# irconde/SSL4POLYP

Hardware: AMD Instinct MI355X
Metric: training-step images/sec/node, ViT-B/16 224^2 (cls fine-tune) (higher is better)
Workload: dtype bf16; 1 GPU; ViT-B/16 classification fine-tune, bs=64/GPU, 224^2, AdamW, random init, finetune mode full (finetune.py:49-91); global_batch=64, parallelism=dp1, launch=eager, lr_schedule=constant

## Files before the change

### ssl4polyp_amd/csrc/pm_attention.hip

```cpp
#include "pm_common.h"
#include <type_traits>

namespace {

template <int DH> constexpr int kTileUnroll = DH == 32 ? 2 : 1;

template <int RB> __device__ __forceinline__ int swz(int row) {
  if constexpr (RB == 64) return (row >> 2) & 3;
  else if constexpr (RB == 128) return (((row >> 1) & 1) << 2) | ((row >> 2) & 3);
  else if constexpr (RB == 384) return row & 7;
  else return row & 15;
}

constexpr int row_bytes_of(int esize, int dh) { return dh == 80 ? (esize == 2 ? 256 : 384) : dh * esize; }
template <typename T, int DH> constexpr int row_bytes() { return row_bytes_of((int)sizeof(T), DH); }

template <typename T, int DH>
__device__ __forceinline__ void load_image(char* img, const T* __restrict__ src, long ld, int rows_valid,
                                           int rows_total, int tid, int nthreads) {
  constexpr int RB = row_bytes<T, DH>();
  constexpr int CPV = DH * sizeof(T) / 16;
  constexpr int CPF = ((DH + 31) / 32) * 32 * sizeof(T) / 16;
  constexpr int EPC = 16 / sizeof(T);
  for (int id = tid; id < rows_total * CPF; id += nthreads) {
    const int row = id / CPF, c = id % CPF;
    u32x4 v = {0u, 0u, 0u, 0u};
    if (row < rows_valid && c < CPV) v = *reinterpret_cast<const u32x4*>(src + (long)row * ld + c * EPC);
    *reinterpret_cast<u32x4*>(img + row * RB + 16 * (c ^ swz<RB>(row))) = v;
  }
}

template <typename T, int DH>
__device__ __forceinline__ Frag16 frag_rows(const char* img, int rb, int kk, int lane) {
  constexpr int RB = row_bytes<T, DH>();
  const int row = rb + (lane & 31);
  const int c = 2 * kk + (lane >> 5);
  Frag16 f;
  f.u = *reinterpret_cast<const u32x4*>(img + row * RB + 16 * (c ^ swz<RB>(row)));
  return f;
}

template <typename T>
__device__ __forceinline__ Frag16 frag_global(const T* __restrict__ rowptr, bool valid, int kk, int lane) {
  constexpr int EPC = 16 / sizeof(T);
  Frag16 f;
  f.u = (u32x4){0u, 0u, 0u, 0u};
  if (valid) f.u = *reinterpret_cast<const u32x4*>(rowptr + (2 * kk + (lane >> 5)) * EPC);
  return f;
}

template <typename T, int DH>
__device__ __forceinline__ f32x16 mma_imgT_acc(const char* PM_LDS_IMAGE img, int rb, int d0, const f32x16& x, f32x16 acc, int lane) {
  constexpr int RB = row_bytes<T, DH>();
  if constexpr (sizeof(T) == 2) {
    const int g = lane >> 4, i = lane & 15, q = i >> 2, p = i & 3, hh = g >> 1;
    const int col = d0 + 16 * (g & 1) + 4 * p;
    const int c = col >> 3, sub = 8 * (p & 1);
    using lds_s4 = __attribute__((address_space(3))) short4v;
#pragma unroll
    for (int s = 0; s < 2; ++s) {
      Frag16 a, b;
      const int r0 = rb + 16 * s + 4 * hh + q;
      const int r1 = r0 + 8;
      const short4v lo = __builtin_amdgcn_ds_read_tr16_b64_v4i16((lds_s4*)(img + r0 * RB + 16 * (c ^ swz<RB>(r0)) + sub));
      const short4v hi = __builtin_amdgcn_ds_read_tr16_b64_v4i16((lds_s4*)(img + r1 * RB + 16 * (c ^ swz<RB>(r1)) + sub));
      a.u[0] = ((unsigned)(unsigned short)lo[0]) | (((unsigned)(unsigned short)lo[1]) << 16);
      a.u[1] = ((unsigned)(unsigned short)lo[2]) | (((unsigned)(unsigned short)lo[3]) << 16);
      a.u[2] = ((unsigned)(unsigned short)hi[0]) | (((unsigned)(unsigned short)hi[1]) << 16);
      a.u[3] = ((unsigned)(unsigned short)hi[2]) | (((unsigned)(unsigned short)hi[3]) << 16);
#pragma unroll
      for (int j = 0; j < 8; ++j) frag_set<T>(b, j, x[8 * s + j]);
      acc = mfma16B<T>(a, b, acc);
    }
  } else {
    const int hh = lane >> 5;
    const int col = d0 + (lane & 31);
#pragma unroll
    for (int r = 0; r < 16; ++r) {
      const int row = rb + acc_row(r, hh);
      const float a = *reinterpret_cast<const float*>(img + row * RB + 16 * ((col >> 2) ^ swz<RB>(row)) + 4 * (col & 3));
      acc = __builtin_amdgcn_mfma_f32_32x32x2f32(a, x[r], acc, 0, 0, 0);
    }
  }
  return acc;
}

__device__ __forceinline__ f32x16 zero16() {
  f32x16 z;
#pragma unroll
  for (int r = 0; r < 16; ++r) z[r] = 0.f;
  return z;
}

template <typename T>
__device__ __forceinline__ void store_tile_T(T* __restrict__ rowptr, bool valid, const f32x16& acc, float scale, int lane,
                                             int ncols = 32) {
  if (!valid) return;
  const int hh = lane >> 5;
#pragma unroll
  for (int g = 0; g < 4; ++g) {
    f32x4 v = {acc[4 * g] * scale, acc[4 * g + 1] * scale, acc[4 * g + 2] * scale, acc[4 * g + 3] * scale};
    if (8 * g + 4 * hh < ncols) store4<T>(rowptr + 8 * g + 4 * hh, v);
  }
}
template <int DH> __device__ __forceinline__ constexpr int tile_cols(int dt) { return DH - 32 * dt < 32 ? DH - 32 * dt : 32; }

constexpr float kLog2e = 1.4426950408889634f;

template <int DH> __device__ __forceinline__ int problem_of_block(int bid, int nprob, int H) {
  if constexpr (DH == 32) {
    if ((nprob & 15) == 0 && (H & 1) == 0) {
      const int xcd = bid & 7, j = bid >> 3;
      return (((j >> 1) << 3) + xcd) * 2 + (j & 1);
    }
  }
  return bid;
}

constexpr int chunk_tiles(int row_bytes, int nt) {
  const int per_tile = 2 * 32 * row_bytes + 2 * 32 * (int)sizeof(float);
  if (nt * per_tile <= 150 * 1024) return nt;
  return (80 * 1024) / per_tile;
}

template <typename T, int DH, int NT, int CT>
__global__ __launch_bounds__(NT * 64) void attn_fwd_kernel(const T* __restrict__ qkv, T* __restrict__ out,
                                                                        float* __restrict__ lse, int N, int H,
                                                                        float scale) {
  constexpr int RB = row_bytes<T, DH>();
  constexpr int KS = DH * sizeof(T) / 32;
  constexpr int DT = (DH + 31) / 32;
  extern __shared__ __attribute__((aligned(16))) char smem[];
  char* imgK = smem;
  char* imgV = smem + CT * 32 * RB;
  const int tid = threadIdx.x, lane = tid & 63, wave = tid >> 6, hh = lane >> 5;
  const int prob = problem_of_block<DH>(blockIdx.x, gridDim.x, H);
  const int b = prob / H, h = prob % H;
  const long ld = 3L * H * DH;
  const T* base = qkv + (long)b * N * ld + h * DH;
  const float c = scale * kLog2e;
  const int q = wave * 32 + (lane & 31);
  const bool qv = q < N;
  Frag16 fq[KS];
  f32x16 o[DT];
#pragma unroll
  for (int dt = 0; dt < DT; ++dt) o[dt] = zero16();
  float m = -INFINITY, l = 0.f;
  for (int c0 = 0; c0 < NT; c0 += CT) {
    if (c0) __syncthreads();
    load_image<T, DH>(imgK, base + H * DH + (long)c0 * 32 * ld, ld, N - c0 * 32, CT * 32, tid, NT * 64);
    load_image<T, DH>(imgV, base + 2 * H * DH + (long)c0 * 32 * ld, ld, N - c0 * 32, CT * 32, tid, NT * 64);
    __syncthreads();
    if (c0 == 0) {
#pragma unroll
      for (int kk = 0; kk < KS; ++kk) fq[kk] = frag_global<T>(base + (long)q * ld, qv, kk, lane);
    }
    const int cend = c0 + CT < NT ? c0 + CT : NT;
#pragma unroll 1
    for (int kt = c0; kt < cend; ++kt) {
      const int rb = (kt - c0) * 32;
      f32x16 s = zero16();
#pragma unroll
      for (int kk = 0; kk < KS; ++kk) s = mfma16B<T>(frag_rows<T, DH>(imgK, rb, kk, lane), fq[kk], s);
      float tm = -INFINITY;
      if (kt * 32 + 32 > N) {
#pragma unroll
        for (int r = 0; r < 16; ++r) {
          const int key = kt * 32 + acc_row(r, hh);
          s[r] = key < N ? s[r] : -INFINITY;
        }
      }
#pragma unroll
      for (int r = 0; r < 16; ++r) tm = fmaxf(tm, s[r]);
      tm = fmaxf(tm, __shfl_xor(tm, 32, 64));
      const float mn = fmaxf(m, tm);
      const float alpha = __builtin_amdgcn_exp2f((m - mn) * c);
      const float mnc = mn * c;
      float ts = 0.f;
#pragma unroll
      for (int r = 0; r < 16; ++r) {
        s[r] = __builtin_amdgcn_exp2f(s[r] * c - mnc);
        ts += s[r];
      }
      l = l * alpha + ts;
      const bool moved = __builtin_amdgcn_ballot_w64(mn != m) != 0;
      m = mn;
#pragma unroll
      for (int dt = 0; dt < DT; ++dt) {
        if (moved) {
#pragma unroll
          for (int r = 0; r < 16; ++r) o[dt][r] *= alpha;
        }
        o[dt] = mma_imgT_acc<T, DH>(imgV, rb, dt * 32, s, o[dt], lane);
      }
    }
  }
  l += __shfl_xor(l, 32, 64);
  if (qv && hh == 0) lse[((long)b * H + h) * N + q] = m * scale + __logf(l);
  const float inv = 1.0f / l;
  T* orow = out + ((long)b * N + q) * H * DH + h * DH;
#pragma unroll
  for (int dt = 0; dt < DT; ++dt) store_tile_T<T>(orow + dt * 32, qv, o[dt], inv, lane, tile_cols<DH>(dt));
}

template <typename T, int DH, int NT, int CT>
__global__ __launch_bounds__(NT * 64) void attn_bwd_q_kernel(const T* __restrict__ qkv, const T* __restrict__ out,
                                                                          const T* __restrict__ dout,
                                                                          const float* __restrict__ lse,
                                                                          float* __restrict__ delta, T* __restrict__ dqkv,
                                                                          int N, int H, float scale) {
  constexpr int RB = row_bytes<T, DH>();
  constexpr int KS = DH * sizeof(T) / 32;
  constexpr int DT = (DH + 31) / 32;
  constexpr int EPC = 16 / sizeof(T);
  extern __shared__ __attribute__((aligned(16))) char smem[];
  char* imgK = smem;
  char* imgV = smem + CT * 32 * RB;
  const int tid = threadIdx.x, lane = tid & 63, wave = tid >> 6, hh = lane >> 5;
  const int prob = problem_of_block<DH>(blockIdx.x, gridDim.x, H);
  const int b = prob / H, h = prob % H;
  const long ld = 3L * H * DH, ldo = (long)H * DH;
  const T* base = qkv + (long)b * N * ld + h * DH;
  const float c = scale * kLog2e;
  const int q = wave * 32 + (lane & 31);
  const bool qv = q < N;
  const long sidx = ((long)b * H + h) * N + q;
  Frag16 fq[KS], fdo[KS];
  float l2 = 0.f, dls = 0.f;
  f32x16 dq[DT];
#pragma unroll
  for (int dt = 0; dt < DT; ++dt) dq[dt] = zero16();
  for (int c0 = 0; c0 < NT; c0 += CT) {
    if (c0) __syncthreads();
    load_image<T, DH>(imgK, base + H * DH + (long)c0 * 32 * ld, ld, N - c0 * 32, CT * 32, tid, NT * 64);
    load_image<T, DH>(imgV, base + 2 * H * DH + (long)c0 * 32 * ld, ld, N - c0 * 32, CT * 32, tid, NT * 64);
    __syncthreads();
    if (c0 == 0) {
      const T* orow = out + ((long)b * N + q) * ldo + h * DH;
      const T* dorow = dout + ((long)b * N + q) * ldo + h * DH;
      float dl = 0.f;
#pragma unroll
      for (int kk = 0; kk < KS; ++kk) {
        fq[kk] = frag_global<T>(base + (long)q * ld, qv, kk, lane);
        fdo[kk] = frag_global<T>(dorow, qv, kk, lane);
        const Frag16 fo = frag_global<T>(orow, qv, kk, lane);
#pragma unroll
        for (int e = 0; e < EPC; ++e) dl += frag_get<T>(fdo[kk], e) * frag_get<T>(fo, e);
      }
      dl += __shfl_xor(dl, 32, 64);
      if (qv && hh == 0) delta[sidx] = dl;
      l2 = qv ? lse[sidx] * kLog2e : 0.f;
      dls = dl * scale;
    }
    const int cend = c0 + CT < NT ? c0 + CT : NT;
#pragma unroll kTileUnroll<DH>
    for (int kt = c0; kt < cend; ++kt) {
      const int rb = (kt - c0) * 32;
      f32x16 s = zero16(), dp = zero16();
#pragma unroll
      for (int kk = 0; kk < KS; ++kk) {
        s = mfma16B<T>(frag_rows<T, DH>(imgK, rb, kk, lane), fq[kk], s);
        dp = mfma16B<T>(frag_rows<T, DH>(imgV, rb, kk, lane), fdo[kk], dp);
      }
#pragma unroll
      for (int r = 0; r < 16; ++r) s[r] = __builtin_amdgcn_exp2f(fminf(s[r] * c - l2, 0.f)) * (dp[r] * scale - dls);
#pragma unroll
      for (int dt = 0; dt < DT; ++dt) dq[dt] = mma_imgT_acc<T, DH>(imgK, rb, dt * 32, s, dq[dt], lane);
    }
  }
  T* dqrow = dqkv + ((long)b * N + q) * ld + h * DH;
#pragma unroll
  for (int dt = 0; dt < DT; ++dt) store_tile_T<T>(dqrow + dt * 32, qv, dq[dt], 1.0f, lane, tile_cols<DH>(dt));
}

template <typename T, int DH, int NT, int CT>
__global__ __launch_bounds__(NT * 64) void attn_bwd_kv_kernel(const T* __restrict__ qkv, const T* __restrict__ dout,
                                                                           const float* __restrict__ lse,
                                                                           const float* __restrict__ delta,
                                                                           T* __restrict__ dqkv, int N, int H, float scale) {
  constexpr int RB = row_bytes<T, DH>();
  constexpr int KS = DH * sizeof(T) / 32;
  constexpr int DT = (DH + 31) / 32;
  extern __shared__ __attribute__((aligned(16))) char smem[];
  char* imgQ = smem;
  char* imgDO = smem + CT * 32 * RB;
  float* sl2 = reinterpret_cast<float*>(smem + 2 * CT * 32 * RB);
  float* sdl = sl2 + CT * 32;
  const int tid = threadIdx.x, lane = tid & 63, wave = tid >> 6, hh = lane >> 5;
  const int prob = problem_of_block<DH>(blockIdx.x, gridDim.x, H);
  const int b = prob / H, h = prob % H;
  const long ld = 3L * H * DH, ldo = (long)H * DH;
  const T* base = qkv + (long)b * N * ld + h * DH;
  const float c = scale * kLog2e;
  const int key = wave * 32 + (lane & 31);
  const bool kv = key < N;
  Frag16 fk[KS], fv[KS];
  f32x16 dk[DT], dv[DT];
#pragma unroll
  for (int dt = 0; dt < DT; ++dt) {
    dk[dt] = zero16();
    dv[dt] = zero16();
  }
  for (int c0 = 0; c0 < NT; c0 += CT) {
    if (c0) __syncthreads();
    load_image<T, DH>(imgQ, base + (long)c0 * 32 * ld, ld, N - c0 * 32, CT * 32, tid, NT * 64);
    load_image<T, DH>(imgDO, dout + ((long)b * N + c0 * 32) * ldo + h * DH, ldo, N - c0 * 32, CT * 32, tid, NT * 64);
    for (int i = tid; i < CT * 32; i += NT * 64) {
      const int qi = c0 * 32 + i;
      const long sidx = ((long)b * H + h) * N + qi;
      sl2[i] = qi < N ? lse[sidx] * kLog2e : 0.f;
      sdl[i] = qi < N ? delta[sidx] * scale : 0.f;
    }
    __syncthreads();
    if (c0 == 0) {
#pragma unroll
      for (int kk = 0; kk < KS; ++kk) {
        fk[kk] = frag_global<T>(base + (long)key * ld + H * DH, kv, kk, lane);
        fv[kk] = frag_global<T>(base + (long)key * ld + 2 * H * DH, kv, kk, lane);
      }
    }
    const int cend = c0 + CT < NT ? c0 + CT : NT;
#pragma unroll kTileUnroll<DH>
    for (int qt = c0; qt < cend; ++qt) {
      const int rb = (qt - c0) * 32;
      f32x16 s = zero16(), dp = zero16();
#pragma unroll
      for (int kk = 0; kk < KS; ++kk) {
        s = mfma16B<T>(frag_rows<T, DH>(imgQ, rb, kk, lane), fk[kk], s);
        dp = mfma16B<T>(frag_rows<T, DH>(imgDO, rb, kk, lane), fv[kk], dp);
      }
#pragma unroll
      for (int g = 0; g < 4; ++g) {
        const int qq = rb + 8 * g + 4 * hh;
        const f32x4 l4 = *reinterpret_cast<const f32x4*>(sl2 + qq);
        const f32x4 d4 = *reinterpret_cast<const f32x4*>(sdl + qq);
#pragma unroll
        for (int e = 0; e < 4; ++e) {
          const int r = 4 * g + e;
          const float p = __builtin_amdgcn_exp2f(fminf(s[r] * c - l4[e], 0.f));
          s[r] = p;
          dp[r] = p * (dp[r] * scale - d4[e]);
        }
      }
#pragma unroll
      for (int dt = 0; dt < DT; ++dt) {
        dv[dt] = mma_imgT_acc<T, DH>(imgDO, rb, dt * 32, s, dv[dt], lane);
        dk[dt] = mma_imgT_acc<T, DH>(imgQ, rb, dt * 32, dp, dk[dt], lane);
      }
    }
  }
  T* drow = dqkv + ((long)b * N + key) * ld + h * DH;
#pragma unroll
  for (int dt = 0; dt < DT; ++dt) {
    store_tile_T<T>(drow + H * DH + dt * 32, kv, dk[dt], 1.0f, lane, tile_cols<DH>(dt));
    store_tile_T<T>(drow + 2 * H * DH + dt * 32, kv, dv[dt], 1.0f, lane, tile_cols<DH>(dt));
  }
}

template <int RB, typename T> __device__ __forceinline__ void dma_rows(char* img, const T* __restrict__ base, long ld, int rows_valid,
                                                                        int piece, int lane) {
  static_assert(sizeof(T) == 2, "16-bit rows");
  constexpr int CPR = RB / 16, RPP = 1024 / RB;
  const int row = piece * RPP + lane / CPR, cs = lane % CPR;
  const int c = cs ^ swz<RB>(row);
  const int gr = row < rows_valid ? row : rows_valid - 1;
  __builtin_amdgcn_global_load_lds((const __attribute__((address_space(1))) void*)(base + (long)gr * ld + c * 8),
                                   (__attribute__((address_space(3))) void*)(img + 1024 * piece), 16, 0, 0);
}

template <typename T, int DH, int NT>
__global__ __launch_bounds__(NT * 64) void attn_fwd2_kernel(const T* __restrict__ qkv, T* __restrict__ out,
                                                           float* __restrict__ lse, int N, int H, int BH, float scale) {
  constexpr int RB = DH * 2;
  constexpr int IMG = NT * 32 * RB;
  constexpr int PCS = IMG / 1024;
  constexpr int KS = RB / 32;
  constexpr int DT = DH / 32;
  extern __shared__ __attribute__((aligned(16))) char smem[];
  char* imgQ = smem + 4 * IMG;
  const int tid = threadIdx.x, lane = tid & 63, hh = lane >> 5;
  const int wave = __builtin_amdgcn_readfirstlane(tid >> 6);
  const long hd = (long)H * DH, ld = 3 * hd;
  const float c = scale * kLog2e;
  auto issue = [&](int head, int buf) {
    const int b = head / H, h = head % H;
    const T* base = qkv + (long)b * N * ld + (long)h * DH;
    char* imgK = smem + buf * 2 * IMG;
#pragma unroll
    for (int i = 0; i < (PCS + NT - 1) / NT; ++i) {
      const int p = wave + NT * i;
      if (p < PCS) {
        dma_rows<RB>(imgK, base + hd, ld, N, p, lane);
        dma_rows<RB>(imgK + IMG, base + 2 * hd, ld, N, p, lane);
        dma_rows<RB>(imgQ, base, ld, N, p, lane);
      }
    }
  };
  int head = blockIdx.x;
  if (head >= BH) return;
  issue(head, 0);
  for (int it = 0; head < BH; head += gridDim.x, ++it) {
    const int buf = it & 1;
    const char* imgK = smem + buf * 2 * IMG;
    const char* imgV = imgK + IMG;
    asm volatile("s_waitcnt vmcnt(0)" ::: "memory");
    __syncthreads();
    Frag16 fq[KS];
#pragma unroll
    for (int kk = 0; kk < KS; ++kk) fq[kk] = frag_rows<T, DH>(imgQ, wave * 32, kk, lane);
    asm volatile("s_waitcnt lgkmcnt(0)" ::: "memory");
    __builtin_amdgcn_sched_barrier(0);
    __syncthreads();
    const int next = head + gridDim.x;
    if (next < BH) issue(next, buf ^ 1);
    const int b = head / H, h = head % H;
    f32x16 s[NT];
#pragma unroll
    for (int kt = 0; kt < NT; ++kt) {
      s[kt] = zero16();
#pragma unroll
      for (int kk = 0; kk < KS; ++kk) s[kt] = mfma16B<T>(frag_rows<T, DH>(imgK, kt * 32, kk, lane), fq[kk], s[kt]);
    }
#pragma unroll
    for (int r = 0; r < 16; ++r) {
      const int key = (NT - 1) * 32 + acc_row(r, hh);
      s[NT - 1][r] = key < N ? s[NT - 1][r] : -INFINITY;
    }
    float m = -INFINITY;
#pragma unroll
    for (int kt = 0; kt < NT; ++kt)
#pragma unroll
      for (int r = 0; r < 16; r += 2) m = fmaxf(m, fmaxf(s[kt][r], s[kt][r + 1]));
    m = fmaxf(m, __shfl_xor(m, 32, 64));
    const float mc = m * c;
    f32x16 o[DT];
#pragma unroll
    for (int dt = 0; dt < DT; ++dt) o[dt] = zero16();
    float l = 0.f;
#pragma unroll
    for (int kt = 0; kt < NT; ++kt) {
#pragma unroll
      for (int r = 0; r < 16; ++r) {
        s[kt][r] = __builtin_amdgcn_exp2f(s[kt][r] * c - mc);
        l += s[kt][r];
      }
#pragma unroll
      for (int dt = 0; dt < DT; ++dt) o[dt] = mma_imgT_acc<T, DH>(imgV, kt * 32, dt * 32, s[kt], o[dt], lane);
    }
    l += __shfl_xor(l, 32, 64);
    const int q = wave * 32 + (lane & 31);
    const bool qv = q < N;
    if (qv && hh == 0) lse[((long)b * H + h) * N + q] = m * scale + __logf(l);
    const float inv = 1.0f / l;
    T* orow = out + ((long)b * N + q) * H * DH + h * DH;
#pragma unroll
    for (int dt = 0; dt < DT; ++dt) store_tile_T<T>(orow + dt * 32, qv, o[dt], inv, lane);
  }
}

template <typename T, int DH, int NT>
__global__ __launch_bounds__(NT * 64) void attn_bwd_fused_kernel(const T* __restrict__ qkv, const T* __restrict__ out,
                                                                const T* __restrict__ dout,
                                                                const float* __restrict__ lse, T* __restrict__ dqkv,
                                                                int N, int H, float scale) {
  constexpr int RB = DH * 2;
  constexpr int IMG = NT * 32 * RB;
  constexpr int PCS = IMG / 1024;
  constexpr int KS = RB / 32;
  constexpr int DT = DH / 32;
  constexpr int CPR = RB / 16;
  extern __shared__ __attribute__((aligned(16))) char smem[];
  char* imgQ = smem;
  char* imgK = smem + IMG;
  char* imgV = smem + 2 * IMG;
  char* imgDO = smem + 3 * IMG;
  float* sl2 = reinterpret_cast<float*>(smem + 4 * IMG);
  float* sdl = sl2 + NT * 32;
  const int tid = threadIdx.x, lane = tid & 63, hh = lane >> 5;
  const int wave = __builtin_amdgcn_readfirstlane(tid >> 6);
  const int prob = problem_of_block<DH>(blockIdx.x, gridDim.x, H);
  const int b = prob / H, h = prob % H;
  const long ld = 3L * H * DH, ldo = (long)H * DH;
  const T* base = qkv + (long)b * N * ld + h * DH;
  const T* dobase = dout + (long)b * N * ldo + h * DH;
#pragma unroll
  for (int i = 0; i < (PCS + NT - 1) / NT; ++i) {
    const int p = wave + NT * i;
    if (p < PCS) {
      dma_rows<RB>(imgQ, base, ld, N, p, lane);
      dma_rows<RB>(imgK, base + H * DH, ld, N, p, lane);
      dma_rows<RB>(imgV, base + 2 * H * DH, ld, N, p, lane);
      dma_rows<RB>(imgDO, dobase, ldo, N, p, lane);
    }
  }
  const int q = wave * 32 + (lane & 31);
  const bool qv = q < N;
  const long sidx = ((long)b * H + h) * N;
  Frag16 fo[KS];
  {
    const T* orow = out + ((long)b * N + (qv ? q : N - 1)) * ldo + h * DH;
#pragma unroll
    for (int kk = 0; kk < KS; ++kk) fo[kk].u = *reinterpret_cast<const u32x4*>(orow + (2 * kk + hh) * 8);
  }
  for (int i = tid; i < NT * 32; i += NT * 64) sl2[i] = i < N ? lse[sidx + i] * kLog2e : 0.f;
  asm volatile("s_waitcnt vmcnt(0)" ::: "memory");
  __syncthreads();
  {
    const int pad0 = N, npad = NT * 32 - N;
    for (int i = tid; i < npad * CPR; i += NT * 64) {
      const int off = (pad0 + i / CPR) * RB + 16 * (i % CPR);
      const u32x4 z = {0u, 0u, 0u, 0u};
      *reinterpret_cast<u32x4*>(imgQ + off) = z;
      *reinterpret_cast<u32x4*>(imgK + off) = z;
      *reinterpret_cast<u32x4*>(imgV + off) = z;
      *reinterpret_cast<u32x4*>(imgDO + off) = z;
    }
  }
  __syncthreads();
  const float c = scale * kLog2e;
  Frag16 fq[KS], fdo[KS];
  float dl = 0.f;
#pragma unroll
  for (int kk = 0; kk < KS; ++kk) {
    fq[kk] = frag_rows<T, DH>(imgQ, wave * 32, kk, lane);
    fdo[kk] = frag_rows<T, DH>(imgDO, wave * 32, kk, lane);
#pragma unroll
    for (int e = 0; e < 8; ++e) dl += frag_get<T>(fdo[kk], e) * frag_get<T>(fo[kk], e);
  }
  dl += __shfl_xor(dl, 32, 64);
  if (!qv) dl = 0.f;
  if (hh == 0) sdl[q] = dl * scale;
  {
    const float l2 = sl2[q];
    const float dls = dl * scale;
    f32x16 dq[DT];
#pragma unroll
    for (int dt = 0; dt < DT; ++dt) dq[dt] = zero16();
#pragma unroll kTileUnroll<DH>
    for (int kt = 0; kt < NT; ++kt) {
      f32x16 s = zero16(), dp = zero16();
#pragma unroll
      for (int kk = 0; kk < KS; ++kk) {
        s = mfma16B<T>(frag_rows<T, DH>(imgK, kt * 32, kk, lane), fq[kk], s);
        dp = mfma16B<T>(frag_rows<T, DH>(imgV, kt * 32, kk, lane), fdo[kk], dp);
      }
#pragma unroll
      for (int r = 0; r < 16; ++r) s[r] = __builtin_amdgcn_exp2f(fminf(s[r] * c - l2, 0.f)) * (dp[r] * scale - dls);
#pragma unroll
      for (int dt = 0; dt < DT; ++dt) dq[dt] = mma_imgT_acc<T, DH>(imgK, kt * 32, dt * 32, s, dq[dt], lane);
    }
    T* dqrow = dqkv + ((long)b * N + q) * ld + h * DH;
#pragma unroll
    for (int dt = 0; dt < DT; ++dt) store_tile_T<T>(dqrow + dt * 32, qv, dq[dt], 1.0f, lane);
  }
  __syncthreads();
  {
    const int key = q;
    const bool kv = qv;
    Frag16 fk[KS], fv[KS];
#pragma unroll
    for (int kk = 0; kk < KS; ++kk) {
      fk[kk] = frag_rows<T, DH>(imgK, wave * 32, kk, lane);
      fv[kk] = frag_rows<T, DH>(imgV, wave * 32, kk, lane);
    }
    f32x16 dk[DT], dv[DT];
#pragma unroll
    for (int dt = 0; dt < DT; ++dt) {
      dk[dt] = zero16();
      dv[dt] = zero16();
    }
#pragma unroll kTileUnroll<DH>
    for (int qt = 0; qt < NT; ++qt) {
      f32x16 s = zero16(), dp = zero16();
#pragma unroll
      for (int kk = 0; kk < KS; ++kk) {
        s = mfma16B<T>(frag_rows<T, DH>(imgQ, qt * 32, kk, lane), fk[kk], s);
        dp = mfma16B<T>(frag_rows<T, DH>(imgDO, qt * 32, kk, lane), fv[kk], dp);
      }
#pragma unroll
      for (int g = 0; g < 4; ++g) {
        const int qq = qt * 32 + 8 * g + 4 * hh;
        const f32x4 l4 = *reinterpret_cast<const f32x4*>(sl2 + qq);
        const f32x4 d4 = *reinterpret_cast<const f32x4*>(sdl + qq);
#pragma unroll
        for (int e = 0; e < 4; ++e) {
          const int r = 4 * g + e;
          const float pr = __builtin_amdgcn_exp2f(fminf(s[r] * c - l4[e], 0.f));
          s[r] = pr;
          dp[r] = pr * (dp[r] * scale - d4[e]);
        }
      }
#pragma unroll
      for (int dt = 0; dt < DT; ++dt) {
        dv[dt] = mma_imgT_acc<T, DH>(imgDO, qt * 32, dt * 32, s, dv[dt], lane);
        dk[dt] = mma_imgT_acc<T, DH>(imgQ, qt * 32, dt * 32, dp, dk[dt], lane);
      }
    }
    T* drow = dqkv + ((long)b * N + key) * ld + h * DH;
#pragma unroll
    for (int dt = 0; dt < DT; ++dt) {
      store_tile_T<T>(drow + H * DH + dt * 32, kv, dk[dt], 1.0f, lane);
      store_tile_T<T>(drow + 2 * H * DH + dt * 32, kv, dv[dt], 1.0f, lane);
    }
  }
}

int plan_attention(bool backward, int B, int N, int H, int dh, int dtype, pm_attention_plan_info* p) {
  if (B <= 0 || N <= 0 || H <= 0) return PM_ESHAPE;
  if (N > 288) return PM_ESHAPE;
  if (dh != 32 && dh != 64 && dh != 80) return PM_ESHAPE;
  if (dtype != PM_BF16 && dtype != PM_F16 && dtype != PM_F32) return PM_EINVAL;
  const int tiles = (N + 31) / 32, BH = B * H;
  const bool half = dtype != PM_F32;
  const int rb = row_bytes_of(half ? 2 : 4, dh);
  p->nt = dh == 80 ? (tiles <= 3 ? 3 : 9) : tiles <= 1 ? 1 : tiles <= 2 ? 2 : tiles <= 7 ? 7 : 9;
  p->ct = p->nt;
  p->grid = BH;
  p->launches = 1;
  p->lds_bytes[1] = 0;
  if (!backward && half && dh == 64 && tiles == 7) {
    p->family = PM_ATTN_FWD_PERSISTENT;
    const int rounds = (BH + 255) / 256;
    p->grid = (BH + rounds - 1) / rounds;
    p->lds_bytes[0] = 5 * 7 * 32 * dh * 2;
  } else if (!backward) {
    p->family = PM_ATTN_FWD_HEAD;
    p->ct = chunk_tiles(rb, p->nt);
    p->lds_bytes[0] = 2 * p->ct * 32 * rb;
  } else if (half && dh != 80) {
    p->family = PM_ATTN_BWD_FUSED;
    p->lds_bytes[0] = 4 * p->nt * 32 * rb + 2 * p->nt * 32 * sizeof(float);
  } else {
    p->family = PM_ATTN_BWD_SPLIT;
    p->launches = 2;
    p->ct = chunk_tiles(rb, p->nt);
    p->lds_bytes[0] = 2 * p->ct * 32 * rb;
    p->lds_bytes[1] = p->lds_bytes[0] + 2 * p->ct * 32 * sizeof(float);
  }
  return PM_OK;
}

template <int N> using Tiles = std::integral_constant<int, N>;
template <int DH, typename F> int with_nt(int nt, F&& f) {
  if constexpr (DH == 80) {
    if (nt == 3) return f(Tiles<3>{});
  } else {
    if (nt == 1) return f(Tiles<1>{});
    if (nt == 2) return f(Tiles<2>{});
    if (nt == 7) return f(Tiles<7>{});
  }
  return nt == 9 ? f(Tiles<9>{}) : PM_ESHAPE;
}

template <typename T, int DH>
int launch_fwd(const pm_attention_plan_info& p, const void* qkv, void* out, float* lse, int B, int N, int H, hipStream_t s) {
  const float scale = 1.0f / sqrtf((float)DH);
  if constexpr (sizeof(T) == 2 && DH == 64) {
    if (p.family == PM_ATTN_FWD_PERSISTENT) {
      auto kern = attn_fwd2_kernel<T, 64, 7>;
      PM_ALLOW_LDS(kern, p.lds_bytes[0]);
      hipLaunchKernelGGL(kern, dim3(p.grid), dim3(7 * 64), p.lds_bytes[0], s, (const T*)qkv, (T*)out, lse, N, H, B * H, scale);
      return pm_check_launch();
    }
  }
  return with_nt<DH>(p.nt, [&](auto nt) {
    constexpr int NT = decltype(nt)::value;
    auto kern = attn_fwd_kernel<T, DH, NT, chunk_tiles(row_bytes<T, DH>(), NT)>;
    PM_ALLOW_LDS(kern, p.lds_bytes[0]);
    hipLaunchKernelGGL(kern, dim3(p.grid), dim3(NT * 64), p.lds_bytes[0], s, (const T*)qkv, (T*)out, lse, N, H, scale);
    return pm_check_launch();
  });
}

template <typename T, int DH>
int launch_bwd(const pm_attention_plan_info& p, const void* qkv, const void* out, const void* dout, const float* lse, float* delta,
               void* dqkv, int B, int N, int H, hipStream_t s) {
  const float scale = 1.0f / sqrtf((float)DH);
  return with_nt<DH>(p.nt, [&](auto nt) {
    constexpr int NT = decltype(nt)::value;
    if constexpr (sizeof(T) == 2 && DH != 80) {
      auto kern = attn_bwd_fused_kernel<T, DH, NT>;
      PM_ALLOW_LDS(kern, p.lds_bytes[0]);
      hipLaunchKernelGGL(kern, dim3(p.grid), dim3(NT * 64), p.lds_bytes[0], s, (const T*)qkv, (const T*)out, (const T*)dout, lse,
                         (T*)dqkv, N, H, scale);
    } else {
      constexpr int CT = chunk_tiles(row_bytes<T, DH>(), NT);
      auto kq = attn_bwd_q_kernel<T, DH, NT, CT>;
      auto kkv = attn_bwd_kv_kernel<T, DH, NT, CT>;
      PM_ALLOW_LDS(kq, p.lds_bytes[0]);
      PM_ALLOW_LDS(kkv, p.lds_bytes[1]);
      hipLaunchKernelGGL(kq, dim3(p.grid), dim3(NT * 64), p.lds_bytes[0], s, (const T*)qkv, (const T*)out, (const T*)dout, lse,
                         delta, (T*)dqkv, N, H, scale);
      hipLaunchKernelGGL(kkv, dim3(p.grid), dim3(NT * 64), p.lds_bytes[1], s, (const T*)qkv, (const T*)dout, lse,
                         (const float*)delta, (T*)dqkv, N, H, scale);
    }
    return pm_check_launch();
  });
}

}

extern "C" int pm_attention_plan(int backward, int B, int N, int H, int dh, int dtype, pm_attention_plan_info* info) {
  if (!info) return PM_EINVAL;
  return plan_attention(backward != 0, B, N, H, dh, dtype, info);
}

extern "C" int pm_attention_fwd(const void* qkv, void* out, float* lse, int B, int N, int H, int dh, int dtype,
                                void* stream) {
  if (!qkv || !out || !lse) return PM_EINVAL;
  pm_attention_plan_info p;
  const int st = plan_attention(false, B, N, H, dh, dtype, &p);
  if (st) return st;
  hipStream_t s = pm_stream(stream);
  PM_DISPATCH_ACT(dtype, T, {
    if (dh == 80) return launch_fwd<T, 80>(p, qkv, out, lse, B, N, H, s);
    return dh == 64 ? launch_fwd<T, 64>(p, qkv, out, lse, B, N, H, s) : launch_fwd<T, 32>(p, qkv, out, lse, B, N, H, s);
  });
}

extern "C" int pm_attention_bwd(const void* qkv, const void* out, const void* dout, const float* lse, float* delta,
                                void* dqkv, int B, int N, int H, int dh, int dtype, void* stream) {
  if (!qkv || !out || !dout || !lse || !delta || !dqkv) return PM_EINVAL;
  pm_attention_plan_info p;
  const int st = plan_attention(true, B, N, H, dh, dtype, &p);
  if (st) return st;
  hipStream_t s = pm_stream(stream);
  PM_DISPATCH_ACT(dtype, T, {
    if (dh == 80) return launch_bwd<T, 80>(p, qkv, out, dout, lse, delta, dqkv, B, N, H, s);
    return dh == 64 ? launch_bwd<T, 64>(p, qkv, out, dout, lse, delta, dqkv, B, N, H, s)
                    : launch_bwd<T, 32>(p, qkv, out, dout, lse, delta, dqkv, B, N, H, s);
  });
}
```

Baseline: 6520 images/sec.

## Software-pipeline fused attention backward loops and coalesce dK/dV stores via LDS

For bf16/f16 with head dim 64 and up to 8 tiles, the dQ and dK/dV loops of the fused attention backward are restructured into a two-stage software pipeline. The next tile's S/dP MFMAs and the K/V or Q/dO fragment loads are interleaved with the current tile's exp2 and gradient MFMAs, with sched_barriers fixing the order. dQ stores now pack results with permlane32 swaps into 16-byte writes. dK/dV are staged through each wave's own rows of the K/V LDS images so global writes are full coalesced rows. The LDS image order is rearranged for that staging, and the mid barrier no longer waits on outstanding global stores. The cost is higher register pressure and more complex scheduling code, and the pipelined path is limited to the dh=64 case.

```diff
diff --git a/ssl4polyp_amd/csrc/pm_attention.hip b/ssl4polyp_amd/csrc/pm_attention.hip
--- a/ssl4polyp_amd/csrc/pm_attention.hip
+++ b/ssl4polyp_amd/csrc/pm_attention.hip
@@ -50,28 +50,37 @@
 }
 
 template <typename T, int DH>
+__device__ __forceinline__ Frag16 imgT_frag(const char* PM_LDS_IMAGE img, int rb, int d0, int s, int lane) {
+  static_assert(sizeof(T) == 2, "16-bit rows");
+  constexpr int RB = row_bytes<T, DH>();
+  const int g = lane >> 4, i = lane & 15, q = i >> 2, p = i & 3, hh = g >> 1;
+  const int col = d0 + 16 * (g & 1) + 4 * p;
+  const int c = col >> 3, sub = 8 * (p & 1);
+  using lds_s4 = __attribute__((address_space(3))) short4v;
+  Frag16 a;
+  const int r0 = rb + 16 * s + 4 * hh + q;
+  const int r1 = r0 + 8;
+  const short4v lo = __builtin_amdgcn_ds_read_tr16_b64_v4i16((lds_s4*)(img + r0 * RB + 16 * (c ^ swz<RB>(r0)) + sub));
+  const short4v hi = __builtin_amdgcn_ds_read_tr16_b64_v4i16((lds_s4*)(img + r1 * RB + 16 * (c ^ swz<RB>(r1)) + sub));
+  a.u[0] = ((unsigned)(unsigned short)lo[0]) | (((unsigned)(unsigned short)lo[1]) << 16);
+  a.u[1] = ((unsigned)(unsigned short)lo[2]) | (((unsigned)(unsigned short)lo[3]) << 16);
+  a.u[2] = ((unsigned)(unsigned short)hi[0]) | (((unsigned)(unsigned short)hi[1]) << 16);
+  a.u[3] = ((unsigned)(unsigned short)hi[2]) | (((unsigned)(unsigned short)hi[3]) << 16);
+  return a;
+}
+template <typename T> __device__ __forceinline__ Frag16 acc_frag(const f32x16& x, int s) {
+  Frag16 b;
+#pragma unroll
+  for (int j = 0; j < 8; ++j) frag_set<T>(b, j, x[8 * s + j]);
+  return b;
+}
+
+template <typename T, int DH>
 __device__ __forceinline__ f32x16 mma_imgT_acc(const char* PM_LDS_IMAGE img, int rb, int d0, const f32x16& x, f32x16 acc, int lane) {
   constexpr int RB = row_bytes<T, DH>();
   if constexpr (sizeof(T) == 2) {
-    const int g = lane >> 4, i = lane & 15, q = i >> 2, p = i & 3, hh = g >> 1;
-    const int col = d0 + 16 * (g & 1) + 4 * p;
-    const int c = col >> 3, sub = 8 * (p & 1);
-    using lds_s4 = __attribute__((address_space(3))) short4v;
-#pragma unroll
-    for (int s = 0; s < 2; ++s) {
-      Frag16 a, b;
-      const int r0 = rb + 16 * s + 4 * hh + q;
-      const int r1 = r0 + 8;
-      const short4v lo = __builtin_amdgcn_ds_read_tr16_b64_v4i16((lds_s4*)(img + r0 * RB + 16 * (c ^ swz<RB>(r0)) + sub));
-      const short4v hi = __builtin_amdgcn_ds_read_tr16_b64_v4i16((lds_s4*)(img + r1 * RB + 16 * (c ^ swz<RB>(r1)) + sub));
-      a.u[0] = ((unsigned)(unsigned short)lo[0]) | (((unsigned)(unsigned short)lo[1]) << 16);
-      a.u[1] = ((unsigned)(unsigned short)lo[2]) | (((unsigned)(unsigned short)lo[3]) << 16);
-      a.u[2] = ((unsigned)(unsigned short)hi[0]) | (((unsigned)(unsigned short)hi[1]) << 16);
-      a.u[3] = ((unsigned)(unsigned short)hi[2]) | (((unsigned)(unsigned short)hi[3]) << 16);
-#pragma unroll
-      for (int j = 0; j < 8; ++j) frag_set<T>(b, j, x[8 * s + j]);
-      acc = mfma16B<T>(a, b, acc);
-    }
+#pragma unroll
+    for (int s = 0; s < 2; ++s) acc = mfma16B<T>(imgT_frag<T, DH>(img, rb, d0, s, lane), acc_frag<T>(x, s), acc);
   } else {
     const int hh = lane >> 5;
     const int col = d0 + (lane & 31);
@@ -101,6 +110,50 @@
   for (int g = 0; g < 4; ++g) {
     f32x4 v = {acc[4 * g] * scale, acc[4 * g + 1] * scale, acc[4 * g + 2] * scale, acc[4 * g + 3] * scale};
     if (8 * g + 4 * hh < ncols) store4<T>(rowptr + 8 * g + 4 * hh, v);
+  }
+}
+template <typename T> __device__ __forceinline__ void tile_chunks(const f32x16& acc, u32x4 (&out)[2]) {
+  static_assert(sizeof(T) == 2, "16-bit outputs");
+  typedef T __attribute__((ext_vector_type(2))) V2;
+  unsigned w[8];
+#pragma unroll
+  for (int j = 0; j < 8; ++j) {
+    const V2 v = {(T)acc[2 * j], (T)acc[2 * j + 1]};
+    w[j] = __builtin_bit_cast(unsigned, v);
+  }
+#pragma unroll
+  for (int j = 0; j < 2; ++j) {
+    const auto lo = __builtin_amdgcn_permlane32_swap(w[4 * j], w[4 * j + 2], false, false);
+    const auto hi = __builtin_amdgcn_permlane32_swap(w[4 * j + 1], w[4 * j + 3], false, false);
+    out[j] = u32x4{lo[0], hi[0], lo[1], hi[1]};
+  }
+}
+template <typename T>
+__device__ __forceinline__ void store_tile_T16(T* __restrict__ rowptr, bool valid, const f32x16& acc, int lane) {
+  u32x4 v[2];
+  tile_chunks<T>(acc, v);
+#pragma unroll
+  for (int j = 0; j < 2; ++j)
+    if (valid) *reinterpret_cast<u32x4*>(rowptr + 16 * j + 8 * (lane >> 5)) = v[j];
+}
+template <typename T, int DH>
+__device__ __forceinline__ void store_tiles_by_rows(char* stage, T* __restrict__ dst, long ld, int rows_valid,
+                                                    const f32x16 (&acc)[DH / 32], int lane) {
+  constexpr int RB = DH * 2, CPR = RB / 16;
+  const int r = lane & 31, hh = lane >> 5;
+#pragma unroll
+  for (int dt = 0; dt < DH / 32; ++dt) {
+    u32x4 v[2];
+    tile_chunks<T>(acc[dt], v);
+#pragma unroll
+    for (int j = 0; j < 2; ++j) *reinterpret_cast<u32x4*>(stage + r * RB + 16 * ((4 * dt + 2 * j + hh) ^ (r & (CPR - 1)))) = v[j];
+  }
+  asm volatile("s_waitcnt lgkmcnt(0)" ::: "memory");
+#pragma unroll
+  for (int i = 0; i < 32 * CPR / 64; ++i) {
+    const int row = (i * 64 + lane) / CPR, ch = lane % CPR;
+    const u32x4 v = *reinterpret_cast<const u32x4*>(stage + row * RB + 16 * (ch ^ (row & (CPR - 1))));
+    if (row < rows_valid) *reinterpret_cast<u32x4*>(dst + row * ld + ch * 8) = v;
   }
 }
 template <int DH> __device__ __forceinline__ constexpr int tile_cols(int dt) { return DH - 32 * dt < 32 ? DH - 32 * dt : 32; }
@@ -458,6 +511,12 @@
   }
 }
 
+__device__ __forceinline__ void barrier_keep_vmcnt() {
+  asm volatile("s_waitcnt lgkmcnt(0)" ::: "memory");
+  __builtin_amdgcn_s_barrier();
+  asm volatile("" ::: "memory");
+}
+
 template <typename T, int DH, int NT>
 __global__ __launch_bounds__(NT * 64) void attn_bwd_fused_kernel(const T* __restrict__ qkv, const T* __restrict__ out,
                                                                 const T* __restrict__ dout,
@@ -469,11 +528,12 @@
   constexpr int KS = RB / 32;
   constexpr int DT = DH / 32;
   constexpr int CPR = RB / 16;
+  constexpr bool kPipelined = DH == 64 && NT <= 8;
   extern __shared__ __attribute__((aligned(16))) char smem[];
   char* imgQ = smem;
-  char* imgK = smem + IMG;
-  char* imgV = smem + 2 * IMG;
-  char* imgDO = smem + 3 * IMG;
+  char* imgDO = smem + IMG;
+  char* imgK = smem + 2 * IMG;
+  char* imgV = smem + 3 * IMG;
   float* sl2 = reinterpret_cast<float*>(smem + 4 * IMG);
   float* sdl = sl2 + NT * 32;
   const int tid = threadIdx.x, lane = tid & 63, hh = lane >> 5;
@@ -519,11 +579,14 @@
   __syncthreads();
   const float c = scale * kLog2e;
   Frag16 fq[KS], fdo[KS];
-  float dl = 0.f;
 #pragma unroll
   for (int kk = 0; kk < KS; ++kk) {
     fq[kk] = frag_rows<T, DH>(imgQ, wave * 32, kk, lane);
     fdo[kk] = frag_rows<T, DH>(imgDO, wave * 32, kk, lane);
+  }
+  float dl = 0.f;
+#pragma unroll
+  for (int kk = 0; kk < KS; ++kk) {
 #pragma unroll
     for (int e = 0; e < 8; ++e) dl += frag_get<T>(fdo[kk], e) * frag_get<T>(fo[kk], e);
   }
@@ -536,27 +599,98 @@
     f32x16 dq[DT];
 #pragma unroll
     for (int dt = 0; dt < DT; ++dt) dq[dt] = zero16();
+    if constexpr (kPipelined) {
+      Frag16 ka[KS], va[KS];
+      auto read_kv = [&](int kt) {
+#pragma unroll
+        for (int kk = 0; kk < KS; ++kk) {
+          ka[kk] = frag_rows<T, DH>(imgK, kt * 32, kk, lane);
+          va[kk] = frag_rows<T, DH>(imgV, kt * 32, kk, lane);
+        }
+      };
+      auto step = [&](f32x16& s, f32x16& dp, int kt, f32x16& sn, f32x16& dpn, auto next) {
+        constexpr bool NEXT = decltype(next)::value;
+        constexpr int EPU = 16 / (2 * KS);
+        const int kt2 = kt + 2 < NT ? kt + 2 : NT - 1;
+        Frag16 a0[DT], a1[DT];
+        if constexpr (NEXT) {
+          sn = zero16();
+          dpn = zero16();
+        }
+#pragma unroll
+        for (int m = 0; m < 2 * KS; ++m) {
+          const int kk = m >> 1;
+          if constexpr (NEXT) {
+            if ((m & 1) == 0) {
+              sn = mfma16B<T>(ka[kk], fq[kk], sn);
+            } else {
+              dpn = mfma16B<T>(va[kk], fdo[kk], dpn);
+              ka[kk] = frag_rows<T, DH>(imgK, kt2 * 32, kk, lane);
+              va[kk] = frag_rows<T, DH>(imgV, kt2 * 32, kk, lane);
+            }
+            __builtin_amdgcn_sched_barrier(0);
+          }
+          if (m == 2 * KS - 1) {
+#pragma unroll
+            for (int dt = 0; dt < DT; ++dt) a0[dt] = imgT_frag<T, DH>(imgK, kt * 32, dt * 32, 0, lane);
+          }
+#pragma unroll
+          for (int r = m * EPU; r < (m + 1) * EPU; ++r)
+            s[r] = __builtin_amdgcn_exp2f(fminf(__builtin_fmaf(s[r], c, -l2), 0.f)) * __builtin_fmaf(dp[r], scale, -dls);
+          __builtin_amdgcn_sched_barrier(0);
+        }
+#pragma unroll
+        for (int dt = 0; dt < DT; ++dt) a1[dt] = imgT_frag<T, DH>(imgK, kt * 32, dt * 32, 1, lane);
+        const Frag16 b0 = acc_frag<T>(s, 0), b1 = acc_frag<T>(s, 1);
+#pragma unroll
+        for (int dt = 0; dt < DT; ++dt) dq[dt] = mfma16B<T>(a0[dt], b0, dq[dt]);
+#pragma unroll
+        for (int dt = 0; dt < DT; ++dt) dq[dt] = mfma16B<T>(a1[dt], b1, dq[dt]);
+        __builtin_amdgcn_sched_barrier(0);
+      };
+      f32x16 sA = zero16(), dpA = zero16(), sB, dpB;
+      read_kv(0);
+#pragma unroll
+      for (int kk = 0; kk < KS; ++kk) {
+        sA = mfma16B<T>(ka[kk], fq[kk], sA);
+        dpA = mfma16B<T>(va[kk], fdo[kk], dpA);
+      }
+      __builtin_amdgcn_sched_barrier(0);
+      read_kv(NT > 1 ? 1 : 0);
+      int kt = 0;
+#pragma unroll 1
+      for (; kt + 2 < NT; kt += 2) {
+        step(sA, dpA, kt, sB, dpB, std::true_type{});
+        step(sB, dpB, kt + 1, sA, dpA, std::true_type{});
+      }
+      if constexpr (NT % 2 == 0) {
+        step(sA, dpA, kt, sB, dpB, std::true_type{});
+        step(sB, dpB, kt + 1, sA, dpA, std::false_type{});
+      } else {
+        step(sA, dpA, kt, sB, dpB, std::false_type{});
+      }
+    } else {
 #pragma unroll kTileUnroll<DH>
-    for (int kt = 0; kt < NT; ++kt) {
-      f32x16 s = zero16(), dp = zero16();
-#pragma unroll
-      for (int kk = 0; kk < KS; ++kk) {
-        s = mfma16B<T>(frag_rows<T, DH>(imgK, kt * 32, kk, lane), fq[kk], s);
-        dp = mfma16B<T>(frag_rows<T, DH>(imgV, kt * 32, kk, lane), fdo[kk], dp);
-      }
-#pragma unroll
-      for (int r = 0; r < 16; ++r) s[r] = __builtin_amdgcn_exp2f(fminf(s[r] * c - l2, 0.f)) * (dp[r] * scale - dls);
-#pragma unroll
-      for (int dt = 0; dt < DT; ++dt) dq[dt] = mma_imgT_acc<T, DH>(imgK, kt * 32, dt * 32, s, dq[dt], lane);
+      for (int kt = 0; kt < NT; ++kt) {
+        f32x16 s = zero16(), dp = zero16();
+#pragma unroll
+        for (int kk = 0; kk < KS; ++kk) {
+          s = mfma16B<T>(frag_rows<T, DH>(imgK, kt * 32, kk, lane), fq[kk], s);
+          dp = mfma16B<T>(frag_rows<T, DH>(imgV, kt * 32, kk, lane), fdo[kk], dp);
+        }
+#pragma unroll
+        for (int r = 0; r < 16; ++r)
+          s[r] = __builtin_amdgcn_exp2f(fminf(__builtin_fmaf(s[r], c, -l2), 0.f)) * __builtin_fmaf(dp[r], scale, -dls);
+#pragma unroll
+        for (int dt = 0; dt < DT; ++dt) dq[dt] = mma_imgT_acc<T, DH>(imgK, kt * 32, dt * 32, s, dq[dt], lane);
+      }
     }
     T* dqrow = dqkv + ((long)b * N + q) * ld + h * DH;
 #pragma unroll
-    for (int dt = 0; dt < DT; ++dt) store_tile_T<T>(dqrow + dt * 32, qv, dq[dt], 1.0f, lane);
-  }
-  __syncthreads();
+    for (int dt = 0; dt < DT; ++dt) store_tile_T16<T>(dqrow + dt * 32, qv, dq[dt], lane);
+  }
+  barrier_keep_vmcnt();
   {
-    const int key = q;
-    const bool kv = qv;
     Frag16 fk[KS], fv[KS];
 #pragma unroll
     for (int kk = 0; kk < KS; ++kk) {
@@ -569,39 +703,139 @@
       dk[dt] = zero16();
       dv[dt] = zero16();
     }
+    if constexpr (kPipelined) {
+      Frag16 qa[KS], da[KS];
+      f32x4 l4, d4;
+      auto read_qdo = [&](int qt) {
+#pragma unroll
+        for (int kk = 0; kk < KS; ++kk) {
+          qa[kk] = frag_rows<T, DH>(imgQ, qt * 32, kk, lane);
+          da[kk] = frag_rows<T, DH>(imgDO, qt * 32, kk, lane);
+        }
+      };
+      auto step = [&](f32x16& s, f32x16& dp, int qt, f32x16& sn, f32x16& dpn, auto next) {
+        constexpr bool NEXT = decltype(next)::value;
+        constexpr int EPU = 16 / (2 * KS), UPG = 4 / EPU;
+        const int qt1 = qt + 1 < NT ? qt + 1 : NT - 1, qt2 = qt + 2 < NT ? qt + 2 : NT - 1;
+        Frag16 av0[DT], ak0[DT], av1[DT], ak1[DT];
+        f32x4 l4n, d4n;
+        if constexpr (NEXT) {
+          sn = zero16();
+          dpn = zero16();
+        }
+#pragma unroll
+        for (int m = 0; m < 2 * KS; ++m) {
+          const int kk = m >> 1;
+          if constexpr (NEXT) {
+            if ((m & 1) == 0) {
+              sn = mfma16B<T>(qa[kk], fk[kk], sn);
+            } else {
+              dpn = mfma16B<T>(da[kk], fv[kk], dpn);
+            }
+            __builtin_amdgcn_sched_barrier(0);
+          }
+          if (m % UPG == 0) {
+            const int g = m / UPG;
+            const int qq = (g < 3 ? qt * 32 + 8 * (g + 1) : qt1 * 32) + 4 * hh;
+            l4n = *reinterpret_cast<const f32x4*>(sl2 + qq);
+            d4n = *reinterpret_cast<const f32x4*>(sdl + qq);
+          }
+          if (m == 2 * KS - 1) {
+#pragma unroll
+            for (int dt = 0; dt < DT; ++dt) {
+              av0[dt] = imgT_frag<T, DH>(imgDO, qt * 32, dt * 32, 0, lane);
+              ak0[dt] = imgT_frag<T, DH>(imgQ, qt * 32, dt * 32, 0, lane);
+            }
+          }
+#pragma unroll
+          for (int r = m * EPU; r < (m + 1) * EPU; ++r) {
+            const float pr = __builtin_amdgcn_exp2f(fminf(__builtin_fmaf(s[r], c, -l4[r & 3]), 0.f));
+            s[r] = pr;
+            dp[r] = pr * __builtin_fmaf(dp[r], scale, -d4[r & 3]);
+          }
+          if (m % UPG == UPG - 1) {
+            l4 = l4n;
+            d4 = d4n;
+          }
+          __builtin_amdgcn_sched_barrier(0);
+        }
+        const Frag16 p0 = acc_frag<T>(s, 0), s0 = acc_frag<T>(dp, 0), p1 = acc_frag<T>(s, 1), s1 = acc_frag<T>(dp, 1);
+#pragma unroll
+        for (int dt = 0; dt < DT; ++dt) {
+          av1[dt] = imgT_frag<T, DH>(imgDO, qt * 32, dt * 32, 1, lane);
+          ak1[dt] = imgT_frag<T, DH>(imgQ, qt * 32, dt * 32, 1, lane);
+        }
+        __builtin_amdgcn_sched_barrier(0);
+#pragma unroll
+        for (int dt = 0; dt < DT; ++dt) {
+          dv[dt] = mfma16B<T>(av0[dt], p0, dv[dt]);
+          dk[dt] = mfma16B<T>(ak0[dt], s0, dk[dt]);
+        }
+        __builtin_amdgcn_sched_barrier(0);
+        if constexpr (NEXT) read_qdo(qt2);
+        __builtin_amdgcn_sched_barrier(0);
+#pragma unroll
+        for (int dt = 0; dt < DT; ++dt) {
+          dv[dt] = mfma16B<T>(av1[dt], p1, dv[dt]);
+          dk[dt] = mfma16B<T>(ak1[dt], s1, dk[dt]);
+        }
+        __builtin_amdgcn_sched_barrier(0);
+      };
+      f32x16 sA = zero16(), dpA = zero16(), sB, dpB;
+      read_qdo(0);
+      l4 = *reinterpret_cast<const f32x4*>(sl2 + 4 * hh);
+      d4 = *reinterpret_cast<const f32x4*>(sdl + 4 * hh);
+#pragma unroll
+      for (int kk = 0; kk < KS; ++kk) {
+        sA = mfma16B<T>(qa[kk], fk[kk], sA);
+        dpA = mfma16B<T>(da[kk], fv[kk], dpA);
+      }
+      __builtin_amdgcn_sched_barrier(0);
+      read_qdo(NT > 1 ? 1 : 0);
+      int qt = 0;
+#pragma unroll 1
+      for (; qt + 2 < NT; qt += 2) {
+        step(sA, dpA, qt, sB, dpB, std::true_type{});
+        step(sB, dpB, qt + 1, sA, dpA, std::true_type{});
+      }
+      if constexpr (NT % 2 == 0) {
+        step(sA, dpA, qt, sB, dpB, std::true_type{});
+        step(sB, dpB, qt + 1, sA, dpA, std::false_type{});
+      } else {
+        step(sA, dpA, qt, sB, dpB, std::false_type{});
+      }
+    } else {
 #pragma unroll kTileUnroll<DH>
-    for (int qt = 0; qt < NT; ++qt) {
-      f32x16 s = zero16(), dp = zero16();
-#pragma unroll
-      for (int kk = 0; kk < KS; ++kk) {
-        s = mfma16B<T>(frag_rows<T, DH>(imgQ, qt * 32, kk, lane), fk[kk], s);
-        dp = mfma16B<T>(frag_rows<T, DH>(imgDO, qt * 32, kk, lane), fv[kk], dp);
-      }
-#pragma unroll
-      for (int g = 0; g < 4; ++g) {
-        const int qq = qt * 32 + 8 * g + 4 * hh;
-        const f32x4 l4 = *reinterpret_cast<const f32x4*>(sl2 + qq);
-        const f32x4 d4 = *reinterpret_cast<const f32x4*>(sdl + qq);
-#pragma unroll
-        for (int e = 0; e < 4; ++e) {
-          const int r = 4 * g + e;
-          const float pr = __builtin_amdgcn_exp2f(fminf(s[r] * c - l4[e], 0.f));
-          s[r] = pr;
-          dp[r] = pr * (dp[r] * scale - d4[e]);
-        }
-      }
-#pragma unroll
-      for (int dt = 0; dt < DT; ++dt) {
-        dv[dt] = mma_imgT_acc<T, DH>(imgDO, qt * 32, dt * 32, s, dv[dt], lane);
-        dk[dt] = mma_imgT_acc<T, DH>(imgQ, qt * 32, dt * 32, dp, dk[dt], lane);
-      }
-    }
-    T* drow = dqkv + ((long)b * N + key) * ld + h * DH;
-#pragma unroll
-    for (int dt = 0; dt < DT; ++dt) {
-      store_tile_T<T>(drow + H * DH + dt * 32, kv, dk[dt], 1.0f, lane);
-      store_tile_T<T>(drow + 2 * H * DH + dt * 32, kv, dv[dt], 1.0f, lane);
-    }
+      for (int qt = 0; qt < NT; ++qt) {
+        f32x16 s = zero16(), dp = zero16();
+#pragma unroll
+        for (int kk = 0; kk < KS; ++kk) {
+          s = mfma16B<T>(frag_rows<T, DH>(imgQ, qt * 32, kk, lane), fk[kk], s);
+          dp = mfma16B<T>(frag_rows<T, DH>(imgDO, qt * 32, kk, lane), fv[kk], dp);
+        }
+#pragma unroll
+        for (int g = 0; g < 4; ++g) {
+          const int qq = qt * 32 + 8 * g + 4 * hh;
+          const f32x4 l4 = *reinterpret_cast<const f32x4*>(sl2 + qq);
+          const f32x4 d4 = *reinterpret_cast<const f32x4*>(sdl + qq);
+#pragma unroll
+          for (int e = 0; e < 4; ++e) {
+            const int r = 4 * g + e;
+            const float pr = __builtin_amdgcn_exp2f(fminf(__builtin_fmaf(s[r], c, -l4[e]), 0.f));
+            s[r] = pr;
+            dp[r] = pr * __builtin_fmaf(dp[r], scale, -d4[e]);
+          }
+        }
+#pragma unroll
+        for (int dt = 0; dt < DT; ++dt) {
+          dv[dt] = mma_imgT_acc<T, DH>(imgDO, qt * 32, dt * 32, s, dv[dt], lane);
+          dk[dt] = mma_imgT_acc<T, DH>(imgQ, qt * 32, dt * 32, dp, dk[dt], lane);
+        }
+      }
+    }
+    T* drow = dqkv + ((long)b * N + wave * 32) * ld + h * DH;
+    store_tiles_by_rows<T, DH>(imgK + wave * 32 * RB, drow + H * DH, ld, N - wave * 32, dk, lane);
+    store_tiles_by_rows<T, DH>(imgV + wave * 32 * RB, drow + 2 * H * DH, ld, N - wave * 32, dv, lane);
   }
 }
 
```

Measured after the change: 6535 images/sec, median of 6. No clear change (+0.2%).
